# NYXFLOWER/TIP

Measured on AMD Instinct MI355X. Metric: D-D edges aggregated/sec (encoder fwd+bwd), higher is better.
Workload: dtype f32; 1 GPU; TIP-cat full encoder, BioSNAP (645 drugs, 19081 proteins, R=1097), 1xMI355X config; mod=cat, directed_dd_edges=8326508, relations=1097, parallelism=single GPU, launch=hipGraph replay of the captured step, rccl_ranks=0

## Files before the change

include/tipk.h:

```cpp
#ifndef TIPK_H
#define TIPK_H

#include <stdint.h>

#ifdef __cplusplus
extern "C" {
#endif

#define TIPK_ABI_VERSION 30

#define TIPK_OK            0
#define TIPK_EINVAL      (-1)
#define TIPK_EUNSUPPORTED (-2)
#define TIPK_EHIP_BASE   (-1000)

typedef void* tipk_stream_t;

int         tipk_abi_version(void);
const char* tipk_strerror(int status);
const char* tipk_build_id(void);
int         tipk_set_option(const char* name, int value);
int         tipk_get_option(const char* name, int* value);
int         tipk_device_info(int device, int* n_cu, int* lds_bytes_per_cu, int* wavefront, char* arch, int arch_len);

// ... 180 lines not shown
                     tipk_stream_t stream);

int tipk_drug_mix_fwd(const float* xd, int64_t ld_xd, const float* d_norm, const float* mean, int64_t ld_mean,
                      const float* w, int p, int q, int64_t rows, int ne, int cat, float* out, int64_t ld_out,
                      tipk_stream_t stream);

int tipk_drug_mix_gather_supported(int p, int q);
int tipk_drug_mix_gather_fwd(const float* xd, int64_t ld_xd, const float* d_norm, const float* h, int64_t ld_h,
                             const int32_t* ptr, const int32_t* src, const float* scale, const int32_t* wg_desc,
                             const int32_t* order , int64_t n_wg,
                             const float* w, int p, int q, int64_t rows, int ne, int cat, float* out, int64_t ld_out,
                             float* mean, tipk_stream_t stream);
int tipk_drug_mix_bwd(const float* g, int64_t ld_g, const float* d_norm, const float* mean, const float* w, int p, int q,
                      int64_t rows, int ne, int cat, float* g_xd, int64_t ld_gxd, float* g_mean, float* g_w,
                      tipk_stream_t stream);

int tipk_drug_mix_gather_xb_supported(int p, int q, int ne, int cat, int n_bases, int d_out);
int tipk_drug_mix_gather_xb_fwd(const float* xd, int64_t ld_xd, const float* d_norm, const float* h, int64_t ld_h,
                                const int32_t* ptr, const int32_t* src, const float* scale, const int32_t* wg_desc,
                                const int32_t* order , int64_t n_wg, const float* w, int p, int q, int64_t rows, int ne, int cat, float* out,
                                int64_t ld_out, float* mean, const float* basis, const float* root, int n_bases, int d_out,
                                float* xb, float* xroot, tipk_stream_t stream);

int tipk_pd_stage_bwd_supported(int p, int q, int64_t rows, int c1);
int tipk_pd_stage_bwd_limits(int* max_rows, int* max_edges);
int tipk_pd_stage_bwd_wh_slabs(void);
int tipk_pd_stage_bwd(const float* g, int64_t ld_g, const float* d_norm, const float* mean, const float* w, int p, int q,
                      int64_t rows, int ne, int cat, float* g_xd, int64_t ld_gxd, float* g_w_slabs,
                      const int32_t* tptr, const int32_t* tdst, const float* tw, int64_t n_src,
                      const int32_t* wg_rows, int64_t n_row_wg,
                      const float* agg, int64_t ld_agg, int c1, const float* w2, int64_t w2_sk, int64_t w2_sn,
                      const float* row_scale, float* gw, int64_t ld_gw, float* dw2_slabs, float* db2_slabs,
                      tipk_stream_t stream);

int tipk_col_sum(const float* in, int64_t ld_in, int64_t rows, int64_t cols,
                 float* scratch, float* out, tipk_stream_t stream);

int tipk_distmult_fwd(const float* z, int64_t n_nodes, int k, const float* rel_w, int64_t n_rel,
                      const void* idx_u, const void* idx_v, int idx_bytes,
                      const void* edge_type, int et_bytes, int64_t n_triples,
                      int sigmoid, float* score, tipk_stream_t stream);

int tipk_distmult_bwd(const float* g_score, const float* score,
                      const float* z, int64_t n_nodes, int k, const float* rel_w, int64_t n_rel,
                      const void* idx_u, const void* idx_v, int idx_bytes,
                      const void* edge_type, int et_bytes, int64_t n_triples,
                      int sigmoid, const int32_t* tasks, int64_t n_tasks,
                      float* g_z, float* g_w, tipk_stream_t stream);

#define TIPK_DM_MODE_BWD 0
#define TIPK_DM_MODE_LOSS 1
#define TIPK_DM_MODE_LOSS_NOGRAD 2
#define TIPK_DM_ROUTE_GENERIC_GLOBAL 0
#define TIPK_DM_ROUTE_GENERIC_LDS 1
#define TIPK_DM_ROUTE_TASK 2
#define TIPK_DM_ROUTE_OBJECTIVE 3
int tipk_distmult_route(int64_t n_nodes, int k, int mode, int has_tasks, int has_workspace, int idx_bytes, int aligned16);

int64_t tipk_distmult_workspace_bytes(int64_t n_nodes, int k, int64_t n_rel);
int tipk_distmult_loss(const float* z, int64_t n_nodes, int k, const float* rel_w, int64_t n_rel,
                       const void* pos_u, const void* pos_v, const void* neg_u, const void* neg_v,
                       int idx_bytes, const void* edge_type, int et_bytes, int64_t n_triples,
                       const int32_t* tasks, int64_t n_tasks,
                       float* loss_out, float* g_z, float* g_w, void* workspace, tipk_stream_t stream);
int tipk_distmult_loss_store(const float* z, int64_t n_nodes, int k, const float* rel_w, int64_t n_rel,
                             const void* pos_u, const void* pos_v, const void* neg_u, const void* neg_v,
// ... 320 lines not shown
```

tip_amd/csrc/tipk_drugmix.hip:

```cpp
#include "tipk_common.h"

namespace {

constexpr int DG_MAX = 64;

struct DgFwdArgs {
    const float* xd; int64_t ld_xd; const float* d_norm;
    const float* h; int64_t ld_h;
    const int32_t* ptr; const int32_t* src; const float* scale;
    const int2* wg;
    const int32_t* order;
    const float* w; int p, q, ne, cat;
    float* out; int64_t ld_out; float* mean;
    int rows;
    const float* basis; const float* root; int n_bases, d_out;
    float* xb;
    float* xroot;
};

constexpr int DG_XMAX = 128;
constexpr int DG_XLD = DG_XMAX + 2;
constexpr int DG_CP = 4;

template <int PL>
__device__ __forceinline__ float dg_row_sum(const float* __restrict__ h, int64_t ld_h, const int32_t* __restrict__ idx, int e0,
                                            int e1, int cc, int lane) {
    constexpr int SLOTS = 64 / PL, STEPS = PL;
    const int s = lane / PL;
    float acc = 0.f;
    int nxt = e0 + lane < e1 ? idx[e0 + lane] : 0;
    for (int b = e0; b < e1; b += 64) {
        const int cur = nxt;
        nxt = b + 64 + lane < e1 ? idx[b + 64 + lane] : 0;
// ... 232 lines not shown
            const float v = a.g[(int64_t)r * a.ld_g + c];
            a.g_xd[(int64_t)r * a.ld_gxd + c] = a.d_norm ? v / a.d_norm[r] : v;
        }
    }
    if (!a.g_mean) return;
    __syncthreads();
    const int tot = a.rows * a.p;
    const int per = (tot + a.n_wg - 1) / a.n_wg;
    const int i1 = (b + 1) * per < tot ? (b + 1) * per : tot;
    for (int i = b * per + t; i < i1; i += 1024) {
        const int r = i / a.p;
        const int c = i - r * a.p;
        const float* gr = a.g + (int64_t)r * a.ld_g + qoff;
        float v = 0.f;
        for (int j = 0; j < a.q; ++j) v = fmaf(gr[j], wl[c * a.q + j], v);
        a.g_mean[i] = v;
    }
}


struct PdBwdArgs {
    DgBwdArgs m;
    const int32_t* tptr; const int32_t* tdst; const float* tw; int n_src;
    const float* agg; int64_t ld_agg; int c1;
    const float* w2; int64_t w2_sk, w2_sn;
    const float* row_scale;
    float* gw; int64_t ld_gw;
    float* dw2; float* db2;
    const int32_t* wg_rows;
    int rows_per_wg;
    int dbg;
};

constexpr int PD_OFF_WH = 0;
constexpr int PD_OFF_W2 = 4096;
constexpr int PD_OFF_GH = 8192;
constexpr int PD_OFF_AGG = 12288;
constexpr int PD_OFF_TQ = 16384;
constexpr int PD_CHUNK_E = 512;
constexpr int PD_PROD = 16384;
constexpr int PD_OFF_PROD = 20480;
constexpr int PD_OFF_EID = PD_OFF_PROD + PD_PROD;
constexpr int PD_ROWS = 4;
constexpr int PD_WH_WGS = 8;
constexpr int PD_LDS = PD_OFF_EID + 2 * PD_CHUNK_E + 128;
static_assert(PD_LDS >= DG_STAGE + 4096 && PD_LDS * 4 <= 160 * 1024, "LDS layout");

template <int PL>
__global__ __launch_bounds__(1024) void pd_stage_bwd_kernel(PdBwdArgs A) {
    __shared__ float sm[PD_LDS];
    const DgBwdArgs& a = A.m;
    const int t = threadIdx.x;
    const int qoff = a.cat ? a.ne : 0;
    if (blockIdx.x < PD_WH_WGS) {
        if (TIPK_DBG(A.dbg & 1)) return;
        const int share = (a.rows + PD_WH_WGS - 1) / PD_WH_WGS;
        const int ra0 = (int)blockIdx.x * share;
        const int ra1 = ra0 + share < a.rows ? ra0 + share : a.rows;
        const int hq = a.q / 2;
        const int kgi = t / a.tp, pt = t % a.tp;
        const int pi = pt / hq, pj = pt % hq;
        const int pw = a.p + a.q;
        float s00 = 0.f, s01 = 0.f, s10 = 0.f, s11 = 0.f;
        const int lr = t / pw, lc = t - lr * pw, lrs = 1024 / pw;
        for (int r0 = ra0; r0 < ra1; r0 += a.tile) {
            const int nr = ra1 - r0 < a.tile ? ra1 - r0 : a.tile;
            __syncthreads();
            if (lr < lrs) {
                const float* src = lc < a.p ? a.mean + (int64_t)r0 * a.p + lc : a.g + (int64_t)r0 * a.ld_g + qoff + (lc - a.p);
                const int64_t ld = lc < a.p ? a.p : a.ld_g;
                int r = lr;
                for (; r + 3 * lrs < nr; r += 4 * lrs) {
                    const float v0 = src[(int64_t)r * ld], v1 = src[(int64_t)(r + lrs) * ld];
                    const float v2 = src[(int64_t)(r + 2 * lrs) * ld], v3 = src[(int64_t)(r + 3 * lrs) * ld];
                    sm[r * pw + lc] = v0; sm[(r + lrs) * pw + lc] = v1;
                    sm[(r + 2 * lrs) * pw + lc] = v2; sm[(r + 3 * lrs) * pw + lc] = v3;
                }
                for (; r < nr; r += lrs) sm[r * pw + lc] = src[(int64_t)r * ld];
            }
            __syncthreads();
            if (kgi < a.kg) {
                const float* mrow = sm + 2 * pi;
                const float* grow = sm + a.p + 2 * pj;
// ... 233 lines not shown
    if (a.kg > 4096 / (p * q)) a.kg = 4096 / (p * q);
    if (a.kg > 16) a.kg = 16;
    if (a.kg < 1) a.kg = 1;
    a.tile = DG_STAGE / (p + q);
    int64_t n_wg = tipk_ceil_div(rows * (int64_t)(ne > p ? ne : p), 1024);
    if (n_wg < 1) n_wg = 1;
    if (n_wg > 240) n_wg = 240;
    a.n_wg = (int)n_wg;
    hipLaunchKernelGGL(drug_mix_bwd_kernel, dim3((unsigned)(1 + n_wg)), dim3(1024), 0, (hipStream_t)stream, a);
    TIPK_RETURN_LAUNCH();
}

extern "C" int tipk_pd_stage_bwd_supported(int p, int q, int64_t rows, int c1) {
    if (!tipk_drug_mix_gather_supported(p, q) || rows <= 0) return 0;
    if (c1 <= 0 || c1 > 64 || (int64_t)p * c1 > 4096) return 0;
    return 1;
}

extern "C" int tipk_pd_stage_bwd_wh_slabs(void) { return PD_WH_WGS; }

extern "C" int tipk_pd_stage_bwd_limits(int* max_rows, int* max_edges) {
    if (max_rows) *max_rows = 16 * PD_ROWS;
    if (max_edges) *max_edges = PD_CHUNK_E;
    return TIPK_OK;
}

extern "C" int tipk_pd_stage_bwd(const float* g, int64_t ld_g, const float* d_norm, const float* mean, const float* w, int p, int q,
                                 int64_t rows, int ne, int cat, float* g_xd, int64_t ld_gxd, float* g_w_slabs,
                                 const int32_t* tptr, const int32_t* tdst, const float* tw, int64_t n_src,
                                 const int32_t* wg_rows, int64_t n_row_wg,
                                 const float* agg, int64_t ld_agg, int c1, const float* w2, int64_t w2_sk, int64_t w2_sn,
                                 const float* row_scale, float* gw, int64_t ld_gw, float* dw2_slabs, float* db2_slabs,
                                 tipk_stream_t stream) {
    if (rows < 0 || ne < 0 || n_src < 0) return TIPK_EINVAL;
    if (!tipk_pd_stage_bwd_supported(p, q, rows, c1) || (!cat && q != ne)) return TIPK_EUNSUPPORTED;
    if (!g || !mean || !w || !g_w_slabs || !tptr || !tdst || !tw || !agg || !w2 || !gw || !dw2_slabs || !db2_slabs || n_src == 0 ||
        !wg_rows || n_row_wg <= 0 || n_row_wg > 0x7fffffLL ||
        rows * (int64_t)(ne + p + q) > 0x7fffffffLL || n_src > 0x7fffffffLL)
        return TIPK_EINVAL;
    PdBwdArgs A;
    DgBwdArgs& a = A.m;
    a.g = g; a.ld_g = ld_g; a.d_norm = d_norm; a.mean = mean; a.w = w; a.p = p; a.q = q; a.ne = ne; a.cat = cat;
    a.g_xd = g_xd; a.ld_gxd = ld_gxd; a.g_mean = nullptr; a.g_w = g_w_slabs;
    a.rows = (int)rows;
    a.tp = p * q / 4;
    a.kg = 1024 / a.tp;
    if (a.kg > 4096 / (p * q)) a.kg = 4096 / (p * q);
    if (a.kg > 16) a.kg = 16;
    if (a.kg < 1) a.kg = 1;
    a.tile = DG_STAGE / (p + q);
    A.rows_per_wg = 16 * PD_ROWS;
    A.wg_rows = wg_rows;
    const int64_t n_wg = n_row_wg;
    a.n_wg = (int)n_wg;
    A.tptr = tptr; A.tdst = tdst; A.tw = tw; A.n_src = (int)n_src;
    A.agg = agg; A.ld_agg = ld_agg; A.c1 = c1; A.w2 = w2; A.w2_sk = w2_sk; A.w2_sn = w2_sn; A.row_scale = row_scale;
    A.gw = gw; A.ld_gw = ld_gw; A.dw2 = dw2_slabs; A.db2 = db2_slabs;
    A.dbg = TIPK_DBG(tipk_option(TIPK_OPT_DM_DEBUG));
    const dim3 grid((unsigned)(PD_WH_WGS + n_wg));
    hipStream_t st = (hipStream_t)stream;
    if (q <= 8) hipLaunchKernelGGL(pd_stage_bwd_kernel<8>, grid, dim3(1024), 0, st, A);
    else if (q <= 16) hipLaunchKernelGGL(pd_stage_bwd_kernel<16>, grid, dim3(1024), 0, st, A);
    else if (q <= 32) hipLaunchKernelGGL(pd_stage_bwd_kernel<32>, grid, dim3(1024), 0, st, A);
    else hipLaunchKernelGGL(pd_stage_bwd_kernel<64>, grid, dim3(1024), 0, st, A);
    TIPK_RETURN_LAUNCH();
}
```

tip_amd/csrc/tipk_encoder.hip:

```cpp
#include <string.h>
#include <algorithm>
#include <map>
#include <new>
#include <string>
#include <vector>
#include "tipk_common.h"
#include "tipk_pairplan.h"

namespace {

constexpr int PAIR_KGROUP = 8;
constexpr int PP_HID1 = 32, PP_HID2 = 16;

inline int64_t align256(int64_t bytes) { return (bytes + 255) / 256 * 256; }
inline int64_t pad_group(int64_t n) { return (n + PAIR_KGROUP - 1) / PAIR_KGROUP * PAIR_KGROUP; }


struct PdCsrH {
    int64_t n_t = 0, n_table = 0;
    std::vector<int32_t> fwd_ptr, fwd_src, fwd_wg, fwd_order, t_ptr, t_dst, t_wg;
    std::vector<float> scale, t_w;
};

std::vector<int32_t> csr_ptr(const std::vector<int64_t>& idx, int64_t n) {
// ... 408 lines not shown
             const EncWs& w, tipk_stream_t s) {
    const tipk_encoder_dims& dm = h->dims;
    const int64_t n = h->n_drug, n_pad = pad_group(n), np = h->n_prot, nr = h->n_rows;
    const int nb = dm.num_base, d1 = dm.n_hid1, d2 = dm.n_hid2, q = dm.prot_drug_dim, ne = dm.n_embed;
    const int cols = dm.cat ? ne + q : ne;
    const int64_t w2_so = p->lin_layout ? 1 : PP_HID1, w2_si = p->lin_layout ? PP_HID2 : 1;
    int st;
    if (!(flags & TIPK_ENCODER_FROM_FWD)) {
        tipk_gemm_desc gd = gdesc(n, d1, cols, w.x0, cols, 1, p->basis1, d1, 1, w.xb1, (int64_t)nb * 32);
        gd.batch = nb; gd.b_sz = (int64_t)cols * d1; gd.c_sz = 32;
        if ((st = tipk_gemm_f32(&gd, s)) != TIPK_OK) return st;
        gd = gdesc(n, d2, d1, w.x1, d1, 1, p->basis2, d2, 1, w.xb2, (int64_t)nb * 32);
        gd.batch = nb; gd.b_sz = (int64_t)d1 * d2; gd.c_sz = 32;
        if ((st = tipk_gemm_f32(&gd, s)) != TIPK_OK) return st;
        const StreamD& c = h->cells_plan;
        if ((st = tipk_stream_gather_two(p->att1, p->att2, nb, h->n_rel, nb, c.n_wg, c.wave_ptr, c.cells, c.ids, c.idx_unit, w.cells1,
                                         w.cells2, nb, s)) != TIPK_OK)
            return st;
    }
    const int64_t lines = n_pad * n, pg_rows = 2 * h->n_alloc + 1;
    tipk_wg_gemm_desc wj[3];
    if ((st = tipk_rgcn_pair_grads(w.cells2, lines, w.xb2, g, d2, n, nb, d2, h->node_desc, h->slots, h->tile_node, h->n_slots, w.dxb2,
                                   n * d2, d2, w.pg2, pg_rows, s)) != TIPK_OK)
        return st;
    dense_jobs(wj, w.x1, n, d1, p->basis2, p->root2, nb, d2, g, w.dxb2, w.x1, w.gx1, gr->basis2, gr->root2);
    if ((st = tipk_gemm_wg_group(wj, 3, nullptr, 0, s)) != TIPK_OK) return st;
    if ((st = tipk_rgcn_pair_grads(w.cells1, lines, w.xb1, w.gx1, d1, n, nb, d1, h->node_desc, h->slots, h->tile_node, h->n_slots, w.dxb1,
                                   n * d1, d1, w.pg1, pg_rows, s)) != TIPK_OK)
        return st;
    const StreamD& ag = h->att_plan;
    if ((st = tipk_stream_gather_parts_two(w.pg1, w.pg2, nb, nb, h->n_alloc, h->part_first, h->part_len, h->wg_part, ag.n_wg, ag.wave_ptr,
                                           ag.cells, ag.ids, ag.idx_unit, ag.zero_ptr, ag.zero_rows, w.att1, w.att2, nb, s)) != TIPK_OK)
        return st;
    const int64_t r = h->n_rel;
    tipk_slab_sum_desc sums[3];
    sums[0] = slab_desc(w.att1, h->n_parts, r * nb, nb, gr->att1);
    sums[1] = slab_desc(w.att2, h->n_parts, r * nb, nb, gr->att2);
    dense_jobs(wj, w.x0, n, cols, p->basis1, p->root1, nb, d1, w.gx1, w.dxb1, nullptr, w.gx0, gr->basis1, gr->root1);
    if ((st = tipk_gemm_wg_group(wj, 3, sums, 2, s)) != TIPK_OK) return st;
    if ((st = tipk_pd_stage_bwd(w.gx0, cols, d_norm, w.mean, p->hgcn_w, PP_HID2, q, n, ne, dm.cat, gr->embed, ne, w.gwh, h->t_ptr, h->t_dst,
                                h->t_w, nr, h->t_wg, h->n_t_wg, w.agg2, PP_HID1, PP_HID1, p->pp_w2, w2_so, w2_si, nullptr, w.gw, PP_HID1,
                                w.dw2, w.db2, s)) != TIPK_OK)
        return st;
    float* g_w2 = p->lin_layout ? gr->pp_w2 : w.gw2;
    sums[0] = slab_desc(w.dw2, h->n_t_wg, (int64_t)PP_HID1 * PP_HID2, PP_HID2, g_w2);
    sums[1] = slab_desc(w.db2, h->n_t_wg, PP_HID2, PP_HID2, gr->pp_b2);
    sums[2] = slab_desc(w.gwh, h->wh_slabs, (int64_t)PP_HID2 * q, q, gr->hgcn_w);
    const GatherD& rb = h->rows_bwd;
    if ((st = tipk_gather_sum_riders(w.gw, PP_HID1, nr, rb.row_id, rb.edge_w, rb.items, rb.n_items, w.gh1, PP_HID1, nullptr, nullptr, 0,
                                     PP_HID1, rb.G, w.h1, PP_HID1, w.parts, sums, 3, s)) != TIPK_OK)
        return st;
    const int64_t part_rows = tipk_ceil_div(rb.n_items, (int64_t)rb.G);
    sums[0] = slab_desc(w.parts, part_rows, PP_HID1, PP_HID1, gr->pp_b1);
    float* g_tab = p->lin_layout ? gr->pp_w1 : w.gtab;
    const GatherD& pb = h->pp_bwd;
    if ((st = tipk_gather_sum_riders(w.gh1, PP_HID1, np, pb.row_id, pb.edge_w, pb.items, pb.n_items, g_tab, PP_HID1, nullptr, nullptr, 0,
                                     PP_HID1, pb.G, nullptr, 0, nullptr, sums, 1, s)) != TIPK_OK)
        return st;
    if (!p->lin_layout) {
        if ((st = tipk_transpose(w.gtab, np, PP_HID1, gr->pp_w1, s)) != TIPK_OK) return st;
        if ((st = tipk_transpose(w.gw2, PP_HID1, PP_HID2, gr->pp_w2, s)) != TIPK_OK) return st;
    }
    return TIPK_OK;
}

bool params_ok(const tipk_encoder_params* p) {
    return p && p->embed && p->pp_w1 && p->pp_b1 && p->pp_w2 && p->pp_b2 && p->hgcn_w && p->basis1 && p->att1 && p->root1 && p->basis2 &&
           p->att2 && p->root2 && (p->lin_layout == 0 || p->lin_layout == 1);
}

bool grads_ok(const tipk_encoder_grads* g) {
    return g && g->embed && g->pp_w1 && g->pp_b1 && g->pp_w2 && g->pp_b2 && g->hgcn_w && g->basis1 && g->att1 && g->root1 && g->basis2 &&
           g->att2 && g->root2;
}

// ... 124 lines not shown
```

tip_amd/csrc/tipk_gather_sum.hip:

```cpp
#include "tipk_common.h"
#include "tipk_slabs.h"

namespace {

constexpr int ITEM_DIRECT = 1;
constexpr int ITEM_PIECE = 2;
constexpr int ITEM_LEADER = 4;
constexpr int ITEM_NULL = 8;

constexpr int GS_RIDERS = 3;
struct Riders {
    int count;
    int first[GS_RIDERS + 1];
    SlabArgs s[GS_RIDERS];
};

struct Epilogue {
    const float* row_scale;
    const float* bias;
    int relu;
    const float* w; int64_t w_so, w_si;
    const float* bias2; int relu2;
    float* out2; int64_t ld_out2;
    const float* gate; int64_t ld_gate;
// ... 307 lines not shown
    const int64_t m = (((int64_t)blockIdx.x * blockDim.x + threadIdx.x) / TIPK_WAVE) * (TIPK_WAVE / L) + lane / L;
    const int col = sub * V;
    if (m >= n_rows || col >= d) return;
    const int row = rows[3 * m + 0], s0 = rows[3 * m + 1], s1 = rows[3 * m + 2];
    Acc<V> acc;
    acc.zero();
    for (int s = s0; s < s1; ++s) acc.add_row(partial + (int64_t)s * d + col);
    acc.epilogue(ep, row, col);
    acc.store(out + (int64_t)row * ld_out + col);
}

template <int V, int L>
int launch_finalize_small(const float* partial, const int32_t* rows, int64_t n_rows, float* out, int64_t ld_out,
                          Epilogue ep, int d, hipStream_t st) {
    const int64_t waves = tipk_ceil_div(n_rows, TIPK_WAVE / L);
    const int64_t blocks = tipk_ceil_div(waves, 4);
    if (blocks > 0x7fffffffLL) return TIPK_EUNSUPPORTED;
    hipLaunchKernelGGL((gather_sum_finalize_small_kernel<V, L>), dim3((unsigned)blocks), dim3(256), 0, st, partial,
                       rows, n_rows, out, ld_out, ep, d);
    TIPK_RETURN_LAUNCH();
}

template <int V, int L>
int launch_gather(const float* table, int64_t ld_table, const int32_t* row_id, const float* edge_w,
                  const int32_t* items, int64_t n_items, float* out, int64_t ld_out, float* partial,
                  Epilogue ep, int d, int group_slots, bool small, hipStream_t st, Riders rd = Riders{}) {
    constexpr int SLOTS = TIPK_WAVE / L;
    const int4* it4 = reinterpret_cast<const int4*>(items);
    if (group_slots > 0) {
        const int threads = group_slots * L;
        if (threads > 1024 || threads % TIPK_WAVE != 0) return TIPK_EUNSUPPORTED;
        const int64_t blocks = tipk_ceil_div(n_items, group_slots);
        if (blocks > 0x7fffffffLL) return TIPK_EUNSUPPORTED;
        const size_t lds = (size_t)threads * sizeof(Acc<V>);
        int64_t grid = blocks;
        if (rd.count > 0) {
            if (threads != 1024) return TIPK_EUNSUPPORTED;
            const int rider_blocks = rd.first[rd.count];
            for (int q = 0; q <= rd.count; ++q) rd.first[q] += (int)blocks;
            grid += rider_blocks;
            if (grid > 0x7fffffffLL) return TIPK_EUNSUPPORTED;
        }
#define TIPK_GS_LAUNCH(W, G, S, GRID, BLOCK, LDS)                                                             \
        hipLaunchKernelGGL((gather_sum_kernel<V, L, W, G, S>), dim3((unsigned)(GRID)), dim3(BLOCK), LDS, st, table, \
                           ld_table, row_id, edge_w, it4, n_items, out, ld_out, partial, ep, d, rd)
        if (ep.colsum) {
            if constexpr (V == 4) {
                if (threads != 1024 || !small) return TIPK_EUNSUPPORTED;
                if (edge_w)
                    hipLaunchKernelGGL((gather_sum_kernel<V, L, true, true, true, -1>), dim3((unsigned)grid), dim3(threads), lds, st, table,
                                       ld_table, row_id, edge_w, it4, n_items, out, ld_out, partial, ep, d, rd);
                else
                    hipLaunchKernelGGL((gather_sum_kernel<V, L, false, true, true, -1>), dim3((unsigned)grid), dim3(threads), lds, st, table,
                                       ld_table, row_id, edge_w, it4, n_items, out, ld_out, partial, ep, d, rd);
                TIPK_RETURN_LAUNCH();
            } else {
                return TIPK_EUNSUPPORTED;
            }
        }
        if (edge_w) { if (small) TIPK_GS_LAUNCH(true, true, true, grid, threads, lds); else TIPK_GS_LAUNCH(true, true, false, grid, threads, lds); }
        else { if (small) TIPK_GS_LAUNCH(false, true, true, grid, threads, lds); else TIPK_GS_LAUNCH(false, true, false, grid, threads, lds); }
        TIPK_RETURN_LAUNCH();
    }
    if (ep.colsum) return TIPK_EUNSUPPORTED;
    if (rd.count > 0) return TIPK_EUNSUPPORTED;
    const int64_t waves = tipk_ceil_div(n_items, SLOTS);
    const int64_t blocks = tipk_ceil_div(waves, 4);
    if (blocks > 0x7fffffffLL) return TIPK_EUNSUPPORTED;
    if (edge_w) { if (small) TIPK_GS_LAUNCH(true, false, true, blocks, 256, 0); else TIPK_GS_LAUNCH(true, false, false, blocks, 256, 0); }
    else { if (small) TIPK_GS_LAUNCH(false, false, true, blocks, 256, 0); else TIPK_GS_LAUNCH(false, false, false, blocks, 256, 0); }
// ... 284 lines not shown
```

tip_amd/csrc/tipk_gemm.hip:

```cpp
#include <stdlib.h>
#include "tipk_common.h"
#include "tipk_slabs.h"

namespace {

typedef float f32x16 __attribute__((ext_vector_type(16)));

constexpr int BK = 32;
constexpr int PAD = 4;

struct GemmArgs {
    int64_t m, n, k, kbatch, ksplit, kchunk;
    const float* a; int64_t a_sm, a_sk, a_sq, a_sz;
    const float* b; int64_t b_sk, b_sn, b_sq, b_sz;
    float* c; int64_t c_sm, c_sz, c_ss;
    const float* c_in; int64_t cin_sm, cin_sz;
    float alpha;
    int relu;
};

typedef unsigned int u32;

__device__ __forceinline__ float ldg(const float* base, u32 byte_off) {
    return *reinterpret_cast<const float*>(reinterpret_cast<const char*>(base) + byte_off);
// ... 474 lines not shown
    float s = 0.f;
    if (i < count) {
        const float* p = in + i;
        int64_t k = j;
        for (; k + 3 * LANES < n_slabs; k += 4 * LANES) {
            const float v0 = p[k * slab_stride], v1 = p[(k + LANES) * slab_stride];
            const float v2 = p[(k + 2 * LANES) * slab_stride], v3 = p[(k + 3 * LANES) * slab_stride];
            s += v0; s += v1; s += v2; s += v3;
        }
        for (; k < n_slabs; k += LANES) s += p[k * slab_stride];
    }
    red[j][e] = s;
    __syncthreads();
    if (j == 0 && i < count) {
        s = red[0][e];
#pragma unroll
        for (int q = 1; q < LANES; ++q) s += red[q][e];
        s *= alpha;
        if (row_scale) s *= row_scale[i / cols];
        if (addend) s += addend[i];
        if (accumulate) s += out[i];
        if (relu) s = fmaxf(s, 0.f);
        out[i] = s;
    }
}

struct SlabGroupArgs {
    int count;
    int first_block[GROUP_MAX + 1];
    SlabArgs s[GROUP_MAX];
};

__global__ __launch_bounds__(1024) void sum_slabs_group_kernel(SlabGroupArgs sa) {
    __shared__ float red[1024];
    SlabArgs a = sa.s[0];
    int first = 0;
#pragma unroll
    for (int q = 1; q < GROUP_MAX; ++q)
        if (q < sa.count && (int)blockIdx.x >= sa.first_block[q]) { a = sa.s[q]; first = sa.first_block[q]; }
    slab_sum_body(a, (int)blockIdx.x - first, red);
}

constexpr int WGK_MAX = 4, WGK_SUMS = 3, WGK_WAVES = 16;
constexpr int WGK_QUARTER_MAX = 128;

struct WgkJob {
    const float* a; int64_t a_sm, a_sk, a_sq, a_sz;
    const float* b; int64_t b_sk, b_sn, b_sq, b_sz;
    const float* a2; int64_t a2_sm, a2_sk;
    const float* b2; int64_t b2_sk, b2_sn;
    float* c; int64_t c_sm, c_sz;
    const float* c_in; int64_t cin_sm, cin_sz;
    const float* gate; int64_t gate_sm, gate_sz;
    int m, n, k, k2, kbatch;
    int mt, nt;
    int tiles_q, n_first, n_kt, per, nw;
    int vec;
    int quarter, pack;
    float alpha; int relu;
};
struct WgkArgs {
    int n_gemm, n_sum;
    int dbg;
    int first[WGK_MAX + WGK_SUMS + 1];
    WgkJob g[WGK_MAX];
    SlabArgs s[WGK_SUMS];
};

template <bool QT, bool VEC>
__device__ __forceinline__ void wgk_body(const WgkJob& g, int local, float* red, int dbg) {
    constexpr int T = QT ? 16 : 32, L = QT ? 8 : 16, G = 32 / L, NACC = QT ? 4 : 16, NB = QT ? 4 : 2;
    typedef float acc_t __attribute__((ext_vector_type(NACC)));
    const int nt_i = local % g.nt, mt_i = (local / g.nt) % g.mt, z = local / (g.nt * g.mt);
    const int t = threadIdx.x, lane = t & 63, row = lane & (T - 1), kg = lane / T;
    const int w = uniform(t >> 6);
    const int m0 = mt_i * T, n0 = nt_i * T;
    const u32 am = (u32)(m0 + row < g.m ? m0 + row : g.m - 1), bn = (u32)(n0 + row < g.n ? n0 + row : g.n - 1);
// ... 398 lines not shown
```

tip_amd/csrc/tipk_slabs.h:

```cpp
#pragma once
#include "tipk_common.h"

namespace {

struct SlabArgs {
    const float* in; int64_t n_slabs, slab_stride, count; float alpha; int accumulate;
    const float* row_scale; int64_t cols; const float* addend; int relu; const float* gate; float* out; int lanes;
};

__device__ __forceinline__ void slab_sum_body(const SlabArgs& a, int block, float* red) {
    const int first = 0;
    const float* __restrict__ in = a.in;
    if (a.lanes == 1) {
        const int64_t i = ((int64_t)(block - first) * 1024 + threadIdx.x) * 4;
        if (i >= a.count) return;
        const float4* p = reinterpret_cast<const float4*>(in + i);
        const int64_t st4 = a.slab_stride / 4;
        float4 s[4];
#pragma unroll
        for (int j = 0; j < 4; ++j) s[j] = make_float4(0.f, 0.f, 0.f, 0.f);
        int64_t k = 0;
        for (; k + 8 <= a.n_slabs; k += 8) {
            float4 v[8];
#pragma unroll
            for (int u = 0; u < 8; ++u) v[u] = p[(k + u) * st4];
#pragma unroll
            for (int u = 0; u < 8; ++u) { s[u & 3].x += v[u].x; s[u & 3].y += v[u].y; s[u & 3].z += v[u].z; s[u & 3].w += v[u].w; }
        }
        {
            float4 v[8];
#pragma unroll
            for (int u = 0; u < 8; ++u) {
                const int64_t kc = k + u < a.n_slabs ? k + u : (a.n_slabs > 0 ? a.n_slabs - 1 : 0);
                v[u] = a.n_slabs > 0 ? p[kc * st4] : make_float4(0.f, 0.f, 0.f, 0.f);
            }
#pragma unroll
            for (int u = 0; u < 8; ++u)
                if (k + u < a.n_slabs) { s[u & 3].x += v[u].x; s[u & 3].y += v[u].y; s[u & 3].z += v[u].z; s[u & 3].w += v[u].w; }
        }
        float r[4] = {((s[0].x + s[1].x) + s[2].x) + s[3].x, ((s[0].y + s[1].y) + s[2].y) + s[3].y,
                      ((s[0].z + s[1].z) + s[2].z) + s[3].z, ((s[0].w + s[1].w) + s[2].w) + s[3].w};
        const float rs = a.row_scale ? a.row_scale[i / a.cols] : 1.f;
        float4 ad = make_float4(0.f, 0.f, 0.f, 0.f), ac = ad, gt = make_float4(1.f, 1.f, 1.f, 1.f);
        if (a.addend) ad = *reinterpret_cast<const float4*>(a.addend + i);
        if (a.accumulate) ac = *reinterpret_cast<const float4*>(a.out + i);
        if (a.gate) gt = *reinterpret_cast<const float4*>(a.gate + i);
// ... 20 lines not shown
        int64_t k = j;
        for (; k + 3 * lanes < a.n_slabs; k += 4 * lanes) {
            const float v0 = p[k * a.slab_stride], v1 = p[(k + lanes) * a.slab_stride];
            const float v2 = p[(k + 2 * lanes) * a.slab_stride], v3 = p[(k + 3 * lanes) * a.slab_stride];
            s += v0; s += v1; s += v2; s += v3;
        }
        for (; k < a.n_slabs; k += lanes) s += p[k * a.slab_stride];
    }
    red[threadIdx.x] = s;
    __syncthreads();
    if (j == 0 && i < a.count) {
        s = red[e];
        for (int q = 1; q < lanes; ++q) s += red[q * epb + e];
        s *= a.alpha;
        if (a.row_scale) s *= a.row_scale[i / a.cols];
        if (a.addend) s += a.addend[i];
        if (a.accumulate) s += a.out[i];
        if (a.relu) s = fmaxf(s, 0.f);
        if (a.gate && !(a.gate[i] > 0.f)) s = 0.f;
        a.out[i] = s;
    }
}

inline int64_t fill_slab_args(const tipk_slab_sum_desc& d, SlabArgs& a, int* rc) {
    *rc = TIPK_OK;
    if (d.n_slabs < 0 || d.count < 0 || (d.row_scale && d.cols <= 0)) { *rc = TIPK_EINVAL; return 0; }
    if (d.count == 0) return 0;
    if (!d.out || (d.n_slabs > 0 && !d.in)) { *rc = TIPK_EINVAL; return 0; }
    a.in = d.in; a.n_slabs = d.n_slabs; a.slab_stride = d.slab_stride; a.count = d.count; a.alpha = d.alpha;
    a.accumulate = d.accumulate; a.row_scale = d.row_scale; a.cols = d.cols; a.addend = d.addend; a.relu = d.relu;
    a.gate = d.gate; a.out = d.out;
    a.lanes = (d.n_slabs >= 32 && tipk_ceil_div(d.count, 64) < 2048) ? 16 : 4;
    const auto al16 = [](const void* q) { return (reinterpret_cast<uintptr_t>(q) & 15) == 0; };
    if (a.lanes == 4 && d.count % 4 == 0 && d.slab_stride % 4 == 0 && al16(d.in) && al16(d.out) && al16(d.addend) &&
        al16(d.gate) && (!d.row_scale || d.cols % 4 == 0) && d.count >= 4096)
        a.lanes = 1;
    return a.lanes == 1 ? tipk_ceil_div(d.count, 4096) : tipk_ceil_div(d.count, 1024 / a.lanes);
}

}
```

tip_amd/encoder.py:

```python
import torch

from . import ops
from ._lib import check, lib, ptr, stream_ptr


class EncoderPlans(object):
    __slots__ = ('pp', 'pp_rows', 'pd', 'dd1', 'dd2', 'cat')

    def __init__(self, pp, pp_rows, pd, dd1, dd2, cat):
        self.pp, self.pp_rows, self.pd, self.dd1, self.dd2, self.cat = pp, pp_rows, pd, dd1, dd2, cat


def _pair_ok(graph, att, basis, n):
    route = ops.rgcn_route(graph, n, basis.shape[1], basis.shape[2], att.shape[1], att.shape[0])
    return route.pair is not None and route.pair_bwd


def usable(plans, xd, w_h, d_norm, c2_weight, c1_bias, c2_bias, basis1, att1, basis2, att2):
    if plans.pp is None or plans.pp_rows is None or plans.pd is None or plans.dd1 is None or plans.dd2 is None:
        return False
    if c1_bias is None or c2_bias is None or not xd.is_cuda:
        return False
    n, ne = xd.shape
    p, q = w_h.shape
    nb, d_in, d1 = basis1.shape
    _, d1b, d2 = basis2.shape
    cols = ne + q if plans.cat else ne
    L = lib()
    if d_in != cols or d1b != d1 or basis2.shape[0] != nb or att1.shape != att2.shape:
        return False
    if not (w_h.is_contiguous() and (d_norm is None or d_norm.is_contiguous()) and basis1.is_contiguous()):
        return False
    if not L.tipk_drug_mix_gather_xb_supported(int(p), int(q), int(ne), int(plans.cat), int(nb), int(d1)):
        return False
    c1 = c2_weight.shape[1]
    if not (c2_weight.t().is_contiguous() and not c2_weight.is_contiguous()):
# ... 1 lines not shown
    if not L.tipk_pd_stage_bwd_supported(int(p), int(q), int(n), int(c1)) or 't_wg' not in plans.pd.pd_csr:
        return False
    if not (ops.gather_sum_lin_supported(c1, p, plans.pp_rows.fwd.group_slots) and ops.gather_sum_epilogue_supported(plans.pp_rows.bwd, c1)
            and ops.gather_sum_epilogue_supported(plans.pp.bwd, c1)):
        return False
    if not (_pair_ok(plans.dd1, att1, basis1, n) and _pair_ok(plans.dd2, att2, basis2, n)):
        return False
    if not ops.pair_cells_partner_ok(plans.dd1, att1, plans.dd2, att2, n):
        return False
    if plans.dd1.pair_bwd is not plans.dd2.pair_bwd:
        return False
    return ops.sum_slabs_xb_supported(d1, d2)


def drug_mix_gather_xb(xd, h, w_h, d_norm, cat, pd_graph, basis, root, xb_nb):
    csr = pd_graph.pd_csr
    n, ne = xd.shape
    p, q = w_h.shape
    nb, cols, d_out = basis.shape
    assert h.shape == (csr['n_src'], p) and csr['fwd_ptr'].numel() == n + 1 and h.stride(1) == 1 and xd.stride(1) == 1
    assert xb_nb.stride()[-2:] == (32, 1) and xb_nb.shape[1] == nb and xb_nb.stride(0) == nb * 32 and xb_nb.shape[0] >= n
    out = torch.empty((n, cols), dtype=torch.float32, device=xd.device)
    mean = torch.empty((n, p), dtype=torch.float32, device=xd.device)
    xroot = torch.empty((n, d_out), dtype=torch.float32, device=xd.device)
    with ops._timed('drug_mix_gather_xb_fwd[%dx%dx%d -> %dx%d]' % (n, p, q, nb, d_out)):
        check(lib().tipk_drug_mix_gather_xb_fwd(ptr(xd), xd.stride(0), ptr(d_norm), ptr(h), h.stride(0), ptr(csr['fwd_ptr']),
                                                ptr(csr['fwd_src']), ptr(csr['scale']), ptr(csr['fwd_wg']), ptr(csr['fwd_order']),
                                                csr['fwd_wg'].shape[0], ptr(w_h), p, q, n, ne, int(cat), ptr(out), out.stride(0), ptr(mean),
                                                ptr(basis), ptr(root), nb, d_out, ptr(xb_nb), ptr(xroot), stream_ptr(xd.device)),
              'tipk_drug_mix_gather_xb_fwd')
    return out, mean, xroot


def pd_stage_bwd(g_x0, d_norm, mean, w_h, ne, cat, pd_graph, agg, w2, row_scale, want_xd=True):
    csr = pd_graph.pd_csr
    n, p = mean.shape
    q = w_h.shape[1]
    n_src, c1 = agg.shape
    assert w2.shape == (p, c1) and g_x0.stride(1) == 1 and agg.stride(1) == 1 and csr['t_ptr'].numel() == n_src + 1
    dev = g_x0.device
    n_slabs = int(csr['t_wg'].numel()) - 1
    g_xd = torch.empty((n, ne), dtype=torch.float32, device=dev) if want_xd else None
    g_w = torch.empty((int(lib().tipk_pd_stage_bwd_wh_slabs()), p, q), dtype=torch.float32, device=dev)
    gw = torch.empty((n_src, c1), dtype=torch.float32, device=dev)
    dw2 = torch.empty((n_slabs, c1, p), dtype=torch.float32, device=dev)
    db2 = torch.empty((n_slabs, p), dtype=torch.float32, device=dev)
    with ops._timed('pd_stage_bwd[%dx%dx%d,rows=%d]' % (n, p, q, n_src)):
        check(lib().tipk_pd_stage_bwd(ptr(g_x0), g_x0.stride(0), ptr(d_norm), ptr(mean), ptr(w_h), p, q, n, ne, int(cat),
                                      ptr(g_xd), g_xd.stride(0) if g_xd is not None else 0, ptr(g_w),
                                      ptr(csr['t_ptr']), ptr(csr['t_dst']), ptr(csr['t_w']), n_src, ptr(csr['t_wg']), n_slabs,
                                      ptr(agg), agg.stride(0), c1, ptr(w2), w2.stride(0), w2.stride(1), ptr(row_scale),
                                      ptr(gw), gw.stride(0), ptr(dw2), ptr(db2), stream_ptr(dev)), 'tipk_pd_stage_bwd')
    return g_xd, ops.slab_job(g_w), gw, ops.slab_job(dw2), ops.slab_job(db2)


def pair_att_gather_two(pb, pg_a, pg_b):
    nb = pg_a.shape[1]
    assert pg_a.shape == pg_b.shape == (2 * pb.n_alloc + 1, nb) and pg_a.is_contiguous() and pg_b.is_contiguous()
    gp = pb.gather
    sa = torch.empty((pb.n_parts, pb.n_rel, nb), dtype=torch.float32, device=pg_a.device)
    sb = torch.empty_like(sa)
    with ops._timed('pair_att_gather2[parts=%d,edges=%d]' % (pb.n_parts, gp.n_edges)):
        check(lib().tipk_stream_gather_parts_two(ptr(pg_a), ptr(pg_b), nb, nb, pb.n_alloc, ptr(pb.part_first), pb.part_len,
                                                 ptr(pb.wg_part), gp.n_wg, ptr(gp.wave_ptr), ptr(gp.cells), ptr(gp.ids), gp.idx_unit,
                                                 ptr(gp.zero_ptr), ptr(gp.zero_rows), ptr(sa), ptr(sb), nb, stream_ptr(pg_a.device)),
              'tipk_stream_gather_parts_two')
    return ops.slab_job(sa), ops.slab_job(sb)


class _EncoderStep(torch.autograd.Function):

    @staticmethod
    def forward(ctx, xd, w1, b1, w2, b2, w_h, d_norm, basis1, att1, root1, basis2, att2, root2, plans):
        f32c = ops._f32c
        xd, w_h = f32c(xd), f32c(w_h).contiguous()
        basis1, att1, root1 = basis1.contiguous(), att1.contiguous(), root1.contiguous()
        basis2, att2, root2 = basis2.contiguous(), att2.contiguous(), root2.contiguous()
        n = xd.shape[0]
        nb, _, d1 = basis1.shape
        d2 = basis2.shape[2]
        dev = xd.device
        g1, g2 = plans.dd1, plans.dd2
        xl = ops.transpose(w1)
        h1 = ops.gather_sum(plans.pp.fwd, xl, row_scale=plans.pp.scale, bias=b1, relu=True)
        agg2, h_prot = ops.gather_sum_lin(plans.pp_rows.fwd, h1, w2, b2, False, row_scale=plans.pp_rows.scale)
# ... 8 lines not shown
        x1 = torch.empty((n, d1), dtype=torch.float32, device=dev)
        xroot2 = ops.sum_slabs_xb(slabs1.view(-1, n, d1), g1.scale, xroot1, True, x1, basis2, root2, xb2)
        pair2 = g2.pair_fwd
        slabs2 = ops.pair_product(cells2, xb2, symmetric=pair2.symmetric, links=getattr(pair2, 'links', None), zeros=zeros2)
        z = ops.sum_slabs(slabs2.view(-1, n, d2), row_scale=g2.scale, addend=xroot2, relu=False)
        ctx.plans, ctx.stamps, ctx.ne = plans, (g1.pair_stamp, g2.pair_stamp), xd.shape[1]
        ctx.save_for_backward(w1, w2, w_h, d_norm, basis1, att1, root1, basis2, att2, root2, h1, agg2, mean, x0, x1)
        return z

    @staticmethod
    def backward(ctx, g):
        w1, w2, w_h, d_norm, basis1, att1, root1, basis2, att2, root2, h1, agg2, mean, x0, x1 = ctx.saved_tensors
        plans = ctx.plans
        g1, g2 = plans.dd1, plans.dd2
        g = ops._f32c(g).contiguous()
        n = x0.shape[0]
        nb, _, d1 = basis1.shape
        d2 = basis2.shape[2]
        dev = g.device
        cells1, xb1, _ = g1.pair_buffers(n, nb, d1, dev)
        cells2, xb2, _ = g2.pair_buffers(n, nb, d2, dev)
        if (g1.pair_stamp, g2.pair_stamp) != ctx.stamps:
            ops.gemm(x0, basis1, out=xb1[:n].permute(1, 0, 2))
            ops.gemm(x1, basis2, out=xb2[:n].permute(1, 0, 2))
            ops.stream_gather_two(g1.pair_fwd, att1, att2, cells1.view(-1, nb)[:n * n], cells2.view(-1, nb)[:n * n])
            g1.pair_stamp += 1
            g2.pair_stamp += 1
            ctx.stamps = (g1.pair_stamp, g2.pair_stamp)
        pb = g1.pair_bwd
        pg2, dxb2 = ops.pair_grads(pb, cells2, xb2, g, table=1)
        g_x1, g_basis2, g_root2 = ops.rgcn_dense_tail(x1, basis2, root2, g, dxb2, x1, [])
        pg1, dxb1 = ops.pair_grads(pb, cells1, xb1, g_x1, table=0)
        j_att1, j_att2 = pair_att_gather_two(pb, pg1, pg2)
        g_x0, g_basis1, g_root1 = ops.rgcn_dense_tail(x0, basis1, root1, g_x1, dxb1, None, [j_att1, j_att2])
        g_xd, j_wh, gw, j_w2, j_b2 = pd_stage_bwd(g_x0, d_norm, mean, w_h, ctx.ne, plans.cat, plans.pd, agg2, w2, plans.pp_rows.scale,
                                                 want_xd=ctx.needs_input_grad[0])
        g_h1, parts = ops.gather_sum(plans.pp_rows.bwd, gw, riders=[j_w2, j_b2, j_wh], gate=h1, colsum=True)
        g_agg = ops.rows_affine(g_h1, row_mul=plans.pp.scale) if plans.pp.scale is not None else g_h1
        j_b1 = ops.slab_job(parts)
        g_table = ops.gather_sum(plans.pp.bwd, g_agg, riders=[j_b1])
        g_w1 = g_table.t() if w1.t().is_contiguous() else ops.transpose(g_table)
        g_w2 = j_w2.out.t()
        return (g_xd, g_w1, j_b1.out.view(-1), g_w2, j_b2.out.view(-1), j_wh.out, None,
                g_basis1, j_att1.out, g_root1, g_basis2, j_att2.out, g_root2, None)


class _PDStage(torch.autograd.Function):

    @staticmethod
    def forward(ctx, h1, w2, b2, xd, w_h, d_norm, pp_rows, pd, cat, link):
        h1, xd, w_h = ops._f32c(h1), ops._f32c(xd), ops._f32c(w_h).contiguous()
        agg2, h_prot = ops.gather_sum_lin(pp_rows.fwd, h1, w2, b2, False, row_scale=pp_rows.scale)
        x0, mean, w_h = ops.drug_mix_gather_launch(xd, h_prot, w_h, d_norm, cat, pd)
        ctx.pp_rows, ctx.pd, ctx.cat, ctx.link, ctx.ne = pp_rows, pd, cat, link, xd.shape[1]
        ctx.save_for_backward(h1, w2, w_h, d_norm, agg2, mean)
        return x0

    @staticmethod
    def backward(ctx, g):
        h1, w2, w_h, d_norm, agg2, mean = ctx.saved_tensors
        pd = ctx.pd
        g = ops._f32c(g)
        g_xd, j_wh, gw, j_w2, j_b2 = pd_stage_bwd(g, d_norm, mean, w_h, ctx.ne, ctx.cat, pd, agg2, w2, ctx.pp_rows.scale,
                                                 want_xd=ctx.needs_input_grad[3])
        want = ctx.link is not None
        res = ops.gather_sum(ctx.pp_rows.bwd, gw, riders=[j_w2, j_b2, j_wh], gate=h1, colsum=want)
        g_h1 = res[0] if want else res
        if want:
            ctx.link.parts = res[1]
# ... 23 lines not shown
```

Measured before the change: 41.46 billion edges/s.

## Move attention slab-sum riders into PD-stage backward kernel and add vec16 slab path

The two attention-gradient slab reductions now run as extra workgroups appended to the pd_stage_bwd launch instead of riding on the dense GEMM group launch. This lets the GEMM group run alone and lets the short slab sums overlap with the longer PD-stage work. A new VEC16 slab-sum path uses float4 loads across 16 slab lanes with an LDS reduction for many-slab, small-count reductions. The GEMM quarter limit is also raised. This adds LDS sizing requirements and more branching at kernel entry.

```diff
diff --git a/include/tipk.h b/include/tipk.h
--- a/include/tipk.h
+++ b/include/tipk.h
@@ -236,6 +236,14 @@
                       const float* agg, int64_t ld_agg, int c1, const float* w2, int64_t w2_sk, int64_t w2_sn,
                       const float* row_scale, float* gw, int64_t ld_gw, float* dw2_slabs, float* db2_slabs,
                       tipk_stream_t stream);
+int tipk_pd_stage_bwd_riders(const float* g, int64_t ld_g, const float* d_norm, const float* mean, const float* w, int p, int q,
+                             int64_t rows, int ne, int cat, float* g_xd, int64_t ld_gxd, float* g_w_slabs,
+                             const int32_t* tptr, const int32_t* tdst, const float* tw, int64_t n_src,
+                             const int32_t* wg_rows, int64_t n_row_wg,
+                             const float* agg, int64_t ld_agg, int c1, const float* w2, int64_t w2_sk, int64_t w2_sn,
+                             const float* row_scale, float* gw, int64_t ld_gw, float* dw2_slabs, float* db2_slabs,
+                             const struct tipk_slab_sum_desc* sums , int32_t n_sums,
+                             tipk_stream_t stream);
 
 int tipk_col_sum(const float* in, int64_t ld_in, int64_t rows, int64_t cols,
                  float* scratch, float* out, tipk_stream_t stream);
diff --git a/tip_amd/csrc/tipk_drugmix.hip b/tip_amd/csrc/tipk_drugmix.hip
--- a/tip_amd/csrc/tipk_drugmix.hip
+++ b/tip_amd/csrc/tipk_drugmix.hip
@@ -1,4 +1,5 @@
 #include "tipk_common.h"
+#include "tipk_slabs.h"
 
 namespace {
 
@@ -297,6 +298,13 @@
     int dbg;
 };
 
+constexpr int PD_RIDERS = 3;
+struct PdRiders {
+    int count;
+    int first[PD_RIDERS + 1];
+    SlabArgs s[PD_RIDERS];
+};
+
 constexpr int PD_OFF_WH = 0;
 constexpr int PD_OFF_W2 = 4096;
 constexpr int PD_OFF_GH = 8192;
@@ -309,11 +317,20 @@
 constexpr int PD_ROWS = 4;
 constexpr int PD_WH_WGS = 8;
 constexpr int PD_LDS = PD_OFF_EID + 2 * PD_CHUNK_E + 128;
-static_assert(PD_LDS >= DG_STAGE + 4096 && PD_LDS * 4 <= 160 * 1024, "LDS layout");
+static_assert(PD_LDS >= DG_STAGE + 4096 && PD_LDS * 4 <= 160 * 1024 && PD_LDS >= SLAB_RED_FLOATS, "LDS layout");
 
 template <int PL>
-__global__ __launch_bounds__(1024) void pd_stage_bwd_kernel(PdBwdArgs A) {
-    __shared__ float sm[PD_LDS];
+__global__ __launch_bounds__(1024) void pd_stage_bwd_kernel(PdBwdArgs A, PdRiders rd) {
+    __shared__ __attribute__((aligned(16))) float sm[PD_LDS];
+    if (rd.count > 0 && (int)blockIdx.x >= rd.first[0]) {
+        SlabArgs sa = rd.s[0];
+        int first = rd.first[0];
+#pragma unroll
+        for (int q = 1; q < PD_RIDERS; ++q)
+            if (q < rd.count && (int)blockIdx.x >= rd.first[q]) { sa = rd.s[q]; first = rd.first[q]; }
+        slab_sum_body(sa, (int)blockIdx.x - first, sm);
+        return;
+    }
     const DgBwdArgs& a = A.m;
     const int t = threadIdx.x;
     const int qoff = a.cat ? a.ne : 0;
@@ -613,6 +630,33 @@
                                  const float* agg, int64_t ld_agg, int c1, const float* w2, int64_t w2_sk, int64_t w2_sn,
                                  const float* row_scale, float* gw, int64_t ld_gw, float* dw2_slabs, float* db2_slabs,
                                  tipk_stream_t stream) {
+    return tipk_pd_stage_bwd_riders(g, ld_g, d_norm, mean, w, p, q, rows, ne, cat, g_xd, ld_gxd, g_w_slabs, tptr, tdst, tw, n_src, wg_rows,
+                                    n_row_wg, agg, ld_agg, c1, w2, w2_sk, w2_sn, row_scale, gw, ld_gw, dw2_slabs, db2_slabs, nullptr, 0,
+                                    stream);
+}
+
+extern "C" int tipk_pd_stage_bwd_riders(const float* g, int64_t ld_g, const float* d_norm, const float* mean, const float* w, int p,
+                                        int q, int64_t rows, int ne, int cat, float* g_xd, int64_t ld_gxd, float* g_w_slabs,
+                                        const int32_t* tptr, const int32_t* tdst, const float* tw, int64_t n_src,
+                                        const int32_t* wg_rows, int64_t n_row_wg,
+                                        const float* agg, int64_t ld_agg, int c1, const float* w2, int64_t w2_sk, int64_t w2_sn,
+                                        const float* row_scale, float* gw, int64_t ld_gw, float* dw2_slabs, float* db2_slabs,
+                                        const tipk_slab_sum_desc* sums, int32_t n_sums, tipk_stream_t stream) {
+    if (n_sums < 0 || n_sums > PD_RIDERS || (n_sums > 0 && !sums)) return TIPK_EINVAL;
+    PdRiders rd;
+    rd.count = 0;
+    int64_t rider_blocks = 0;
+    for (int i = 0; i < n_sums; ++i) {
+        int rc;
+        const int64_t nb = fill_slab_args(sums[i], rd.s[rd.count], &rc);
+        if (rc != TIPK_OK) return rc;
+        if (nb == 0) continue;
+        rd.first[rd.count] = (int)rider_blocks;
+        rider_blocks += nb;
+        if (rider_blocks > 0x3fffffffLL) return TIPK_EUNSUPPORTED;
+        ++rd.count;
+    }
+    for (int i = rd.count; i <= PD_RIDERS; ++i) rd.first[i] = (int)rider_blocks;
     if (rows < 0 || ne < 0 || n_src < 0) return TIPK_EINVAL;
     if (!tipk_pd_stage_bwd_supported(p, q, rows, c1) || (!cat && q != ne)) return TIPK_EUNSUPPORTED;
     if (!g || !mean || !w || !g_w_slabs || !tptr || !tdst || !tw || !agg || !w2 || !gw || !dw2_slabs || !db2_slabs || n_src == 0 ||
@@ -638,11 +682,13 @@
     A.agg = agg; A.ld_agg = ld_agg; A.c1 = c1; A.w2 = w2; A.w2_sk = w2_sk; A.w2_sn = w2_sn; A.row_scale = row_scale;
     A.gw = gw; A.ld_gw = ld_gw; A.dw2 = dw2_slabs; A.db2 = db2_slabs;
     A.dbg = TIPK_DBG(tipk_option(TIPK_OPT_DM_DEBUG));
-    const dim3 grid((unsigned)(PD_WH_WGS + n_wg));
+    const int stage_wgs = PD_WH_WGS + (int)n_wg;
+    for (int i = 0; i <= PD_RIDERS; ++i) rd.first[i] += stage_wgs;
+    const dim3 grid((unsigned)(stage_wgs + rider_blocks));
     hipStream_t st = (hipStream_t)stream;
-    if (q <= 8) hipLaunchKernelGGL(pd_stage_bwd_kernel<8>, grid, dim3(1024), 0, st, A);
-    else if (q <= 16) hipLaunchKernelGGL(pd_stage_bwd_kernel<16>, grid, dim3(1024), 0, st, A);
-    else if (q <= 32) hipLaunchKernelGGL(pd_stage_bwd_kernel<32>, grid, dim3(1024), 0, st, A);
-    else hipLaunchKernelGGL(pd_stage_bwd_kernel<64>, grid, dim3(1024), 0, st, A);
+    if (q <= 8) hipLaunchKernelGGL(pd_stage_bwd_kernel<8>, grid, dim3(1024), 0, st, A, rd);
+    else if (q <= 16) hipLaunchKernelGGL(pd_stage_bwd_kernel<16>, grid, dim3(1024), 0, st, A, rd);
+    else if (q <= 32) hipLaunchKernelGGL(pd_stage_bwd_kernel<32>, grid, dim3(1024), 0, st, A, rd);
+    else hipLaunchKernelGGL(pd_stage_bwd_kernel<64>, grid, dim3(1024), 0, st, A, rd);
     TIPK_RETURN_LAUNCH();
 }
diff --git a/tip_amd/csrc/tipk_encoder.hip b/tip_amd/csrc/tipk_encoder.hip
--- a/tip_amd/csrc/tipk_encoder.hip
+++ b/tip_amd/csrc/tipk_encoder.hip
@@ -464,15 +464,15 @@
     if ((st = tipk_stream_gather_parts_two(w.pg1, w.pg2, nb, nb, h->n_alloc, h->part_first, h->part_len, h->wg_part, ag.n_wg, ag.wave_ptr,
                                            ag.cells, ag.ids, ag.idx_unit, ag.zero_ptr, ag.zero_rows, w.att1, w.att2, nb, s)) != TIPK_OK)
         return st;
+    dense_jobs(wj, w.x0, n, cols, p->basis1, p->root1, nb, d1, w.gx1, w.dxb1, nullptr, w.gx0, gr->basis1, gr->root1);
+    if ((st = tipk_gemm_wg_group(wj, 3, nullptr, 0, s)) != TIPK_OK) return st;
     const int64_t r = h->n_rel;
     tipk_slab_sum_desc sums[3];
     sums[0] = slab_desc(w.att1, h->n_parts, r * nb, nb, gr->att1);
     sums[1] = slab_desc(w.att2, h->n_parts, r * nb, nb, gr->att2);
-    dense_jobs(wj, w.x0, n, cols, p->basis1, p->root1, nb, d1, w.gx1, w.dxb1, nullptr, w.gx0, gr->basis1, gr->root1);
-    if ((st = tipk_gemm_wg_group(wj, 3, sums, 2, s)) != TIPK_OK) return st;
-    if ((st = tipk_pd_stage_bwd(w.gx0, cols, d_norm, w.mean, p->hgcn_w, PP_HID2, q, n, ne, dm.cat, gr->embed, ne, w.gwh, h->t_ptr, h->t_dst,
-                                h->t_w, nr, h->t_wg, h->n_t_wg, w.agg2, PP_HID1, PP_HID1, p->pp_w2, w2_so, w2_si, nullptr, w.gw, PP_HID1,
-                                w.dw2, w.db2, s)) != TIPK_OK)
+    if ((st = tipk_pd_stage_bwd_riders(w.gx0, cols, d_norm, w.mean, p->hgcn_w, PP_HID2, q, n, ne, dm.cat, gr->embed, ne, w.gwh, h->t_ptr,
+                                       h->t_dst, h->t_w, nr, h->t_wg, h->n_t_wg, w.agg2, PP_HID1, PP_HID1, p->pp_w2, w2_so, w2_si, nullptr,
+                                       w.gw, PP_HID1, w.dw2, w.db2, sums, 2, s)) != TIPK_OK)
         return st;
     float* g_w2 = p->lin_layout ? gr->pp_w2 : w.gw2;
     sums[0] = slab_desc(w.dw2, h->n_t_wg, (int64_t)PP_HID1 * PP_HID2, PP_HID2, g_w2);
diff --git a/tip_amd/csrc/tipk_gather_sum.hip b/tip_amd/csrc/tipk_gather_sum.hip
--- a/tip_amd/csrc/tipk_gather_sum.hip
+++ b/tip_amd/csrc/tipk_gather_sum.hip
@@ -363,10 +363,11 @@
         if (threads > 1024 || threads % TIPK_WAVE != 0) return TIPK_EUNSUPPORTED;
         const int64_t blocks = tipk_ceil_div(n_items, group_slots);
         if (blocks > 0x7fffffffLL) return TIPK_EUNSUPPORTED;
-        const size_t lds = (size_t)threads * sizeof(Acc<V>);
+        size_t lds = (size_t)threads * sizeof(Acc<V>);
         int64_t grid = blocks;
         if (rd.count > 0) {
             if (threads != 1024) return TIPK_EUNSUPPORTED;
+            if (lds < SLAB_RED_FLOATS * sizeof(float)) lds = SLAB_RED_FLOATS * sizeof(float);
             const int rider_blocks = rd.first[rd.count];
             for (int q = 0; q <= rd.count; ++q) rd.first[q] += (int)blocks;
             grid += rider_blocks;
diff --git a/tip_amd/csrc/tipk_gemm.hip b/tip_amd/csrc/tipk_gemm.hip
--- a/tip_amd/csrc/tipk_gemm.hip
+++ b/tip_amd/csrc/tipk_gemm.hip
@@ -530,7 +530,7 @@
 };
 
 __global__ __launch_bounds__(1024) void sum_slabs_group_kernel(SlabGroupArgs sa) {
-    __shared__ float red[1024];
+    __shared__ __attribute__((aligned(16))) float red[SLAB_RED_FLOATS];
     SlabArgs a = sa.s[0];
     int first = 0;
 #pragma unroll
@@ -540,7 +540,7 @@
 }
 
 constexpr int WGK_MAX = 4, WGK_SUMS = 3, WGK_WAVES = 16;
-constexpr int WGK_QUARTER_MAX = 128;
+constexpr int WGK_QUARTER_MAX = 192;
 
 struct WgkJob {
     const float* a; int64_t a_sm, a_sk, a_sq, a_sz;
diff --git a/tip_amd/csrc/tipk_slabs.h b/tip_amd/csrc/tipk_slabs.h
--- a/tip_amd/csrc/tipk_slabs.h
+++ b/tip_amd/csrc/tipk_slabs.h
@@ -5,13 +5,58 @@
 
 struct SlabArgs {
     const float* in; int64_t n_slabs, slab_stride, count; float alpha; int accumulate;
-    const float* row_scale; int64_t cols; const float* addend; int relu; const float* gate; float* out; int lanes;
+    const float* row_scale; int64_t cols; const float* addend; int relu; const float* gate; float* out;
+    int lanes;
 };
+constexpr int SLAB_VEC4 = 1, SLAB_VEC16 = 2;
+constexpr int SLAB_RED_FLOATS = 4096;
 
 __device__ __forceinline__ void slab_sum_body(const SlabArgs& a, int block, float* red) {
     const int first = 0;
     const float* __restrict__ in = a.in;
-    if (a.lanes == 1) {
+    if (a.lanes == SLAB_VEC16) {
+        const int e4 = threadIdx.x & 63, j = threadIdx.x >> 6;
+        const int64_t i = (int64_t)(block - first) * 256 + e4 * 4;
+        float4 s = make_float4(0.f, 0.f, 0.f, 0.f);
+        if (i < a.count) {
+            const float4* p = reinterpret_cast<const float4*>(in + i);
+            const int64_t st4 = a.slab_stride / 4;
+            int64_t k = j;
+            for (; k + 48 < a.n_slabs; k += 64) {
+                const float4 v0 = p[k * st4], v1 = p[(k + 16) * st4], v2 = p[(k + 32) * st4], v3 = p[(k + 48) * st4];
+                s.x += v0.x; s.y += v0.y; s.z += v0.z; s.w += v0.w;
+                s.x += v1.x; s.y += v1.y; s.z += v1.z; s.w += v1.w;
+                s.x += v2.x; s.y += v2.y; s.z += v2.z; s.w += v2.w;
+                s.x += v3.x; s.y += v3.y; s.z += v3.z; s.w += v3.w;
+            }
+            if (k < a.n_slabs) {
+                float4 v[3];
+#pragma unroll
+                for (int u = 0; u < 3; ++u) v[u] = p[(k + 16 * u < a.n_slabs ? k + 16 * u : k) * st4];
+#pragma unroll
+                for (int u = 0; u < 3; ++u)
+                    if (k + 16 * u < a.n_slabs) { s.x += v[u].x; s.y += v[u].y; s.z += v[u].z; s.w += v[u].w; }
+            }
+        }
+        *reinterpret_cast<float4*>(red + j * 256 + e4 * 4) = s;
+        __syncthreads();
+        const int e = threadIdx.x;
+        const int64_t o = (int64_t)(block - first) * 256 + e;
+        if (e < 256 && o < a.count) {
+            float t = red[e];
+#pragma unroll
+            for (int q = 1; q < 16; ++q) t += red[q * 256 + e];
+            t *= a.alpha;
+            if (a.row_scale) t *= a.row_scale[o / a.cols];
+            if (a.addend) t += a.addend[o];
+            if (a.accumulate) t += a.out[o];
+            if (a.relu) t = fmaxf(t, 0.f);
+            if (a.gate && !(a.gate[o] > 0.f)) t = 0.f;
+            a.out[o] = t;
+        }
+        return;
+    }
+    if (a.lanes == SLAB_VEC4) {
         const int64_t i = ((int64_t)(block - first) * 1024 + threadIdx.x) * 4;
         if (i >= a.count) return;
         const float4* p = reinterpret_cast<const float4*>(in + i);
@@ -98,10 +143,13 @@
     a.gate = d.gate; a.out = d.out;
     a.lanes = (d.n_slabs >= 32 && tipk_ceil_div(d.count, 64) < 2048) ? 16 : 4;
     const auto al16 = [](const void* q) { return (reinterpret_cast<uintptr_t>(q) & 15) == 0; };
-    if (a.lanes == 4 && d.count % 4 == 0 && d.slab_stride % 4 == 0 && al16(d.in) && al16(d.out) && al16(d.addend) &&
-        al16(d.gate) && (!d.row_scale || d.cols % 4 == 0) && d.count >= 4096)
-        a.lanes = 1;
-    return a.lanes == 1 ? tipk_ceil_div(d.count, 4096) : tipk_ceil_div(d.count, 1024 / a.lanes);
+    const bool vec = d.count % 4 == 0 && d.slab_stride % 4 == 0 && al16(d.in) && al16(d.out) && al16(d.addend) && al16(d.gate) &&
+                     (!d.row_scale || d.cols % 4 == 0);
+    if (a.lanes == 4 && vec && d.count >= 4096) a.lanes = SLAB_VEC4;
+    else if (a.lanes == 16 && vec) a.lanes = SLAB_VEC16;
+    if (a.lanes == SLAB_VEC4) return tipk_ceil_div(d.count, 4096);
+    if (a.lanes == SLAB_VEC16) return tipk_ceil_div(d.count, 256);
+    return tipk_ceil_div(d.count, 1024 / a.lanes);
 }
 
 }
diff --git a/tip_amd/encoder.py b/tip_amd/encoder.py
--- a/tip_amd/encoder.py
+++ b/tip_amd/encoder.py
@@ -1,7 +1,7 @@
 import torch
 
 from . import ops
-from ._lib import check, lib, ptr, stream_ptr
+from ._lib import SlabSumDesc, check, lib, ptr, stream_ptr
 
 
 class EncoderPlans(object):
@@ -69,7 +69,7 @@
     return out, mean, xroot
 
 
-def pd_stage_bwd(g_x0, d_norm, mean, w_h, ne, cat, pd_graph, agg, w2, row_scale, want_xd=True):
+def pd_stage_bwd(g_x0, d_norm, mean, w_h, ne, cat, pd_graph, agg, w2, row_scale, want_xd=True, riders=()):
     csr = pd_graph.pd_csr
     n, p = mean.shape
     q = w_h.shape[1]
@@ -82,12 +82,15 @@
     gw = torch.empty((n_src, c1), dtype=torch.float32, device=dev)
     dw2 = torch.empty((n_slabs, c1, p), dtype=torch.float32, device=dev)
     db2 = torch.empty((n_slabs, p), dtype=torch.float32, device=dev)
-    with ops._timed('pd_stage_bwd[%dx%dx%d,rows=%d]' % (n, p, q, n_src)):
-        check(lib().tipk_pd_stage_bwd(ptr(g_x0), g_x0.stride(0), ptr(d_norm), ptr(mean), ptr(w_h), p, q, n, ne, int(cat),
-                                      ptr(g_xd), g_xd.stride(0) if g_xd is not None else 0, ptr(g_w),
-                                      ptr(csr['t_ptr']), ptr(csr['t_dst']), ptr(csr['t_w']), n_src, ptr(csr['t_wg']), n_slabs,
-                                      ptr(agg), agg.stride(0), c1, ptr(w2), w2.stride(0), w2.stride(1), ptr(row_scale),
-                                      ptr(gw), gw.stride(0), ptr(dw2), ptr(db2), stream_ptr(dev)), 'tipk_pd_stage_bwd')
+    riders = list(riders)
+    arr = (SlabSumDesc * max(1, len(riders)))(*[r.desc for r in riders])
+    with ops._timed('pd_stage_bwd[%dx%dx%d,rows=%d]' % (n, p, q, n_src) + ('+%d sums' % len(riders) if riders else '')):
+        check(lib().tipk_pd_stage_bwd_riders(ptr(g_x0), g_x0.stride(0), ptr(d_norm), ptr(mean), ptr(w_h), p, q, n, ne, int(cat),
+                                             ptr(g_xd), g_xd.stride(0) if g_xd is not None else 0, ptr(g_w),
+                                             ptr(csr['t_ptr']), ptr(csr['t_dst']), ptr(csr['t_w']), n_src, ptr(csr['t_wg']), n_slabs,
+                                             ptr(agg), agg.stride(0), c1, ptr(w2), w2.stride(0), w2.stride(1), ptr(row_scale),
+                                             ptr(gw), gw.stride(0), ptr(dw2), ptr(db2), arr if riders else None, len(riders),
+                                             stream_ptr(dev)), 'tipk_pd_stage_bwd_riders')
     return g_xd, ops.slab_job(g_w), gw, ops.slab_job(dw2), ops.slab_job(db2)
 
 
@@ -162,9 +165,9 @@
         g_x1, g_basis2, g_root2 = ops.rgcn_dense_tail(x1, basis2, root2, g, dxb2, x1, [])
         pg1, dxb1 = ops.pair_grads(pb, cells1, xb1, g_x1, table=0)
         j_att1, j_att2 = pair_att_gather_two(pb, pg1, pg2)
-        g_x0, g_basis1, g_root1 = ops.rgcn_dense_tail(x0, basis1, root1, g_x1, dxb1, None, [j_att1, j_att2])
+        g_x0, g_basis1, g_root1 = ops.rgcn_dense_tail(x0, basis1, root1, g_x1, dxb1, None, [])
         g_xd, j_wh, gw, j_w2, j_b2 = pd_stage_bwd(g_x0, d_norm, mean, w_h, ctx.ne, plans.cat, plans.pd, agg2, w2, plans.pp_rows.scale,
-                                                 want_xd=ctx.needs_input_grad[0])
+                                                 want_xd=ctx.needs_input_grad[0], riders=[j_att1, j_att2])
         g_h1, parts = ops.gather_sum(plans.pp_rows.bwd, gw, riders=[j_w2, j_b2, j_wh], gate=h1, colsum=True)
         g_agg = ops.rows_affine(g_h1, row_mul=plans.pp.scale) if plans.pp.scale is not None else g_h1
         j_b1 = ops.slab_job(parts)
```

Result: faster. 42.84 billion edges/s (median of 6 runs) (+3.3%).
